# joesound212985/Deepfake-Detection-using-CLIP-Based-SigLIP-2-Vision-Transformers

Hardware: AMD Instinct MI355X
Metric: images/sec (train fwd+bwd) SigLIP-2-so400m@384 bf16 (higher is better)
Workload: dtype bf16; 1 GPU; so400m-patch14-384 encoder+pool-head train fwd+bwd, 384x384, per-GPU batch 128, seeded random weights; global_batch=128, parallelism=dp1

## Files before the change

### deepfake-detection-using-clip-based-siglip-2-vision-transformers_amd/csrc/attention.hip

```cpp
#include <stdlib.h>

#include "common.hip.h"
#include "kernels.h"

namespace sgl {

hipError_t attn_f32_fwd(const float*, const float*, const float*, float*, float*, int, int, int, int, int, int, hipStream_t);
hipError_t attn_f32_bwd(const float*, const float*, const float*, const float*, const float*, const float*, float*,
                        float*, int, int, int, int, int, int, hipStream_t);
hipError_t attn_ref_fwd(const float*, const float*, const float*, float*, float*, int, int, int, int, int, int, hipStream_t);
hipError_t attn_ref_bwd(const float*, const float*, const float*, const float*, const float*, const float*, float*,
                        float*, int, int, int, int, int, int, hipStream_t);

template <int DP>
struct AttnCfg {
  static constexpr int KS = DP / 16;
  static constexpr int DT = (DP + 31) / 32;
  static constexpr int CPR = DP / 8;
  static constexpr int RSTR = DP * 2 + 16;
  static constexpr int TSTR = 192;
  static constexpr int DSTR = 208;
};

__device__ __forceinline__ u32x4 a_ldg(__amdgpu_buffer_rsrc_t r, uint32_t off) {
  return __builtin_amdgcn_raw_buffer_load_b128(r, off, 0, 0);
}
template <typename T>
__device__ __forceinline__ lo_x8<T> as_x8(u32x4 v) { return __builtin_bit_cast(lo_x8<T>, v); }
template <typename T>
__device__ __forceinline__ lo_x8<T> lds_row8(const char* p) { return *reinterpret_cast<const lo_x8<T>*>(p); }
template <typename T>
__device__ __forceinline__ lo_x4<T> lds_tr4(const char* p) { return lds_read_tr16<T>(p); }
template <typename T>
__device__ __forceinline__ lo_x8<T> lds_trfrag(const char* img, int stride, int kk, int dcol0, int lane) {
  const int g = lane >> 4, q = (lane >> 2) & 3, p = lane & 3;
  const char* a = img + (16 * kk + 4 * (g >> 1) + q) * stride + (dcol0 + 16 * (g & 1) + 4 * p) * 2;
  const lo_x4<T> lo = lds_tr4<T>(a);
  const lo_x4<T> hi = lds_tr4<T>(a + 8 * stride);
  return __builtin_shufflevector(lo, hi, 0, 1, 2, 3, 4, 5, 6, 7);
}
template <typename T>
__device__ __forceinline__ lo_x8<T> pack8(const f32x16& s, int base) {
  lo_x8<T> r;
#pragma unroll
  for (int j = 0; j < 8; ++j) r[j] = (T)s[base + j];
  return r;
}
__device__ __forceinline__ float fast_exp2(float x) { return __builtin_amdgcn_exp2f(x); }

__device__ __forceinline__ bool head_block(int nb, int BH, int& bh, int& xb) {
  const int pid = blockIdx.x, xcd = pid & 7, slot = pid >> 3;
  const int hq = slot / nb;
  bh = hq * 8 + xcd;
  xb = slot - hq * nb;
  return bh < BH;
}
static inline dim3 head_grid(int nb, int BH) { return dim3((unsigned)(8 * ((BH + 7) / 8) * nb)); }

struct HeadSrc {
  uint32_t rowbytes, nc, bytes;
  size_t base;
};
__device__ __forceinline__ HeadSrc head_src(int ld, int b, int hd, int H, int N, int dh, int DP) {
  HeadSrc r;
  if (ld > 0) {
    r.rowbytes = (uint32_t)ld * 2u;
    r.nc = (uint32_t)dh / 8u;
    r.bytes = (uint32_t)(((size_t)(N - 1) * ld + dh) * 2);
    r.base = (size_t)b * N * ld + (size_t)hd * dh;
  } else {
    r.rowbytes = (uint32_t)DP * 2u;
    r.nc = (uint32_t)DP / 8u;
    r.bytes = (uint32_t)((size_t)N * DP * 2);
    r.base = ((size_t)b * H + hd) * (size_t)N * DP;
  }
  return r;
}

#define MFMA32(a, b, c) mfma_32x32x16((a), (b), (c))

__device__ __forceinline__ void att_dma16(u32x4 desc, uint32_t lds_addr, uint32_t voff) {
  asm volatile("s_mov_b32 m0, %0\n\ts_nop 0\n\tbuffer_load_dwordx4 %1, %2, 0 offen lds" ::"s"(lds_addr), "v"(voff), "s"(desc)
               : "memory");
}
__device__ __forceinline__ void att_dma4(u32x4 desc, uint32_t lds_addr, uint32_t voff) {
  asm volatile("s_mov_b32 m0, %0\n\ts_nop 0\n\tbuffer_load_dword %1, %2, 0 offen lds" ::"s"(lds_addr), "v"(voff), "s"(desc)
               : "memory");
}
__device__ __forceinline__ u32x4 att_desc(const void* base, uint32_t bytes) {
  const uint64_t q = (uint64_t)base;
  return u32x4{(uint32_t)q, (uint32_t)(q >> 32) & 0xffffu, bytes, 0x00020000u};
}
__device__ __forceinline__ uint32_t att_chunk_off(int cidx, int rows, int SC, int NC, uint32_t rowbytes) {
  const int row = cidx / SC, col = cidx - row * SC;
  return (row < rows && col < NC) ? (uint32_t)row * rowbytes + (uint32_t)col * 16u : SGL_OOB;
}
#define SGL_ATT_WAIT_BARRIER(n)                                   \
  do {                                                            \
    asm volatile("s_waitcnt vmcnt(" #n ") lgkmcnt(0)" ::: "memory"); \
    __builtin_amdgcn_sched_barrier(0);                            \
    __builtin_amdgcn_s_barrier();                                 \
    __builtin_amdgcn_sched_barrier(0);                            \
    asm volatile("" ::: "memory");                                \
  } while (0)

template <typename T, int DP, bool TOK>
__global__ __launch_bounds__(256) __attribute__((amdgpu_waves_per_eu(3, 3))) void attn_fwd_kernel(const T* __restrict__ Q, const T* __restrict__ K,
                                                          const T* __restrict__ V, T* __restrict__ out,
                                                          float* __restrict__ lse, int B, int H, int N, int dh, int ld,
                                                          float c, float scale) {
  using C = AttnCfg<DP>;
  constexpr int KT = 64;
  constexpr int KBYTES = KT * C::RSTR, VBYTES = KT * C::TSTR, STAGE = KBYTES + VBYTES;
  constexpr int SCK = C::RSTR / 16, SCV = C::TSTR / 16;
  constexpr int NIK = KT * SCK / 64, NIV = KT * SCV / 64, NSLOT = NIK + NIV;
  constexpr int NPW = (NSLOT + 3) / 4;
  static_assert(KT * SCK % 64 == 0 && KT * SCV % 64 == 0, "whole DMA instructions per image");
  extern __shared__ __attribute__((aligned(16))) char smem[];
  const int t = threadIdx.x, lane = t & 63;
  const int w = __builtin_amdgcn_readfirstlane(t >> 6);
  int bh, xb;
  if (!head_block((N + 127) / 128, B * H, bh, xb)) return;
  const int b = bh / H, hd = bh - b * H;
  const int q0 = xb * 128 + w * 32;
  HeadSrc src = head_src(TOK ? ld : 0, b, hd, H, N, dh, DP);
  if constexpr (!TOK) {
    src.rowbytes = (uint32_t)DP * 2u;
    src.nc = (uint32_t)DP / 8u;
  }
  const __amdgpu_buffer_rsrc_t rq = make_rsrc(Q + src.base, src.bytes);
  const u32x4 dk_ = att_desc(K + src.base, src.bytes);
  const u32x4 dv_ = att_desc(V + src.base, src.bytes);
  const uint32_t lds0 = (uint32_t)(size_t)((SGL_LDS char*)smem);

  const int qi = lane & 31, hh = lane >> 5;
  lo_x8<T> qf[C::KS];
#pragma unroll
  for (int ks = 0; ks < C::KS; ++ks) {
    const uint32_t ch = (uint32_t)(2 * ks + hh);
    qf[ks] = as_x8<T>(a_ldg(rq, (q0 + qi < N && ch < src.nc) ? (uint32_t)(q0 + qi) * src.rowbytes + ch * 16u : SGL_OOB));
  }

  uint32_t voff[NPW];
#pragma unroll
  for (int j = 0; j < NPW; ++j) {
    const int sl = w + 4 * j;
    voff[j] = (sl < NIK) ? att_chunk_off(sl * 64 + lane, KT, SCK, (int)src.nc, src.rowbytes)
                         : att_chunk_off((sl - NIK) * 64 + lane, KT, SCV, (int)src.nc, src.rowbytes);
  }
  const uint32_t tile_adv = (uint32_t)KT * src.rowbytes;
  auto issue = [&](int stage) {
    const uint32_t sb = lds0 + (uint32_t)(stage * STAGE);
#pragma unroll
    for (int j = 0; j < NPW; ++j) {
      const int sl = w + 4 * j;
      if (sl < NSLOT) att_dma16(sl < NIK ? dk_ : dv_, sb + (uint32_t)sl * 1024u, voff[j]);
      voff[j] += tile_adv;
    }
  };

  float m_run = -INFINITY, l_run = 0.f;
  f32x16 o[C::DT];
#pragma unroll
  for (int dt = 0; dt < C::DT; ++dt)
#pragma unroll
    for (int r = 0; r < 16; ++r) o[dt][r] = 0.f;

  const int ntiles = (N + KT - 1) / KT;
#pragma unroll
  for (int ks = 0; ks < C::KS; ++ks) asm volatile("" ::"v"(qf[ks]));
  asm volatile("s_waitcnt vmcnt(0)" ::: "memory");
  issue(0);
  for (int tile = 0; tile < ntiles; ++tile) {
    const int cur = tile & 1;
    SGL_ATT_WAIT_BARRIER(0);
    if (tile + 1 < ntiles) issue(cur ^ 1);
    const char* kb = smem + cur * STAGE;
    const char* vb = kb + KBYTES;
    f32x16 s0, s1;
#pragma unroll
    for (int r = 0; r < 16; ++r) { s0[r] = 0.f; s1[r] = 0.f; }
#pragma unroll
    for (int ks = 0; ks < C::KS; ++ks) {
      const lo_x8<T> k0 = lds_row8<T>(kb + qi * C::RSTR + (16 * ks + 8 * hh) * 2);
      const lo_x8<T> k1 = lds_row8<T>(kb + (qi + 32) * C::RSTR + (16 * ks + 8 * hh) * 2);
      s0 = MFMA32(k0, qf[ks], s0);
      s1 = MFMA32(k1, qf[ks], s1);
    }
    if (tile == ntiles - 1) {
#pragma unroll
      for (int r = 0; r < 16; ++r) {
        const int key = tile * KT + (r & 3) + 8 * (r >> 2) + 4 * hh;
        if (key >= N) s0[r] = -INFINITY;
        if (key + 32 >= N) s1[r] = -INFINITY;
      }
    }
    float mx = s0[0];
#pragma unroll
    for (int r = 1; r < 16; ++r) mx = fmaxf(mx, s0[r]);
#pragma unroll
    for (int r = 0; r < 16; ++r) mx = fmaxf(mx, s1[r]);
    mx = fmaxf(mx, __shfl_xor(mx, 32, 64));
    const float m_new = fmaxf(m_run, mx);
    const bool grew = __any(m_new > m_run);
    const float alpha = grew ? fast_exp2(c * (m_run - m_new)) : 1.0f;
    const float mc = m_new * c;
    float rs = 0.f;
#pragma unroll
    for (int r = 0; r < 16; ++r) {
      s0[r] = fast_exp2(fmaf(s0[r], c, -mc));
      s1[r] = fast_exp2(fmaf(s1[r], c, -mc));
      rs += s0[r] + s1[r];
    }
    l_run = l_run * alpha + rs;
    m_run = m_new;
    if (grew) {
#pragma unroll
      for (int dt = 0; dt < C::DT; ++dt)
#pragma unroll
        for (int r = 0; r < 16; ++r) o[dt][r] *= alpha;
    }
    lo_x8<T> pb[4];
    pb[0] = pack8<T>(s0, 0);
    pb[1] = pack8<T>(s0, 8);
    pb[2] = pack8<T>(s1, 0);
    pb[3] = pack8<T>(s1, 8);
#pragma unroll
    for (int dt = 0; dt < C::DT; ++dt)
#pragma unroll
      for (int kk = 0; kk < 4; ++kk) o[dt] = MFMA32(lds_trfrag<T>(vb, C::TSTR, kk, dt * 32, lane), pb[kk], o[dt]);
  }
  const float l = l_run + __shfl_xor(l_run, 32, 64);
  const float inv = 1.0f / l;
  const int q = q0 + qi;
  if (q < N) {
    T* orow = out + ((size_t)b * N + q) * ((size_t)H * dh) + hd * dh;
#pragma unroll
    for (int dt = 0; dt < C::DT; ++dt)
#pragma unroll
      for (int g4 = 0; g4 < 4; ++g4) {
        const int d = dt * 32 + 8 * g4 + 4 * hh;
        if (d < dh) {
          lo_x4<T> v4;
#pragma unroll
          for (int r = 0; r < 4; ++r) v4[r] = (T)(o[dt][4 * g4 + r] * inv);
          *reinterpret_cast<lo_x4<T>*>(orow + d) = v4;
        }
      }
    if (hh == 0) lse[(size_t)bh * N + q] = m_run * scale + __logf(l);
  }
}

template <typename T, int DP, bool TOK>
__global__ __launch_bounds__(256, 2) void attn_bwd_kv_kernel(const T* __restrict__ Q, const T* __restrict__ K,
                                                             const T* __restrict__ V, const T* __restrict__ dO,
                                                             const float* __restrict__ aux, T* __restrict__ dqkv,
                                                             int B, int H, int N, int dh, int ld, float c, float scale) {
  using C = AttnCfg<DP>;
  constexpr int QT = 32;
  constexpr int SC = C::DSTR / 16;
  constexpr int NIS = (QT * SC + 63) / 64;
  constexpr int IMG = NIS * 1024;
  constexpr int STAGE = 2 * IMG + QT * 8;
  constexpr int NSLOT = 2 * NIS + 1;
  static_assert(NSLOT <= 16 && NSLOT > 12, "four DMA slots per wave (three for the last wave)");
  extern __shared__ __attribute__((aligned(16))) char smem[];
  const int t = threadIdx.x, lane = t & 63;
  const int w = __builtin_amdgcn_readfirstlane(t >> 6);
  int bh, xb;
  if (!head_block((N + 127) / 128, B * H, bh, xb)) return;
  const int b = bh / H, hd = bh - b * H;
  const int D = H * dh;
  const int key0 = xb * 128 + w * 32;
  HeadSrc src = head_src(TOK ? ld : 0, b, hd, H, N, dh, DP);
  if constexpr (!TOK) {
    src.rowbytes = (uint32_t)DP * 2u;
    src.nc = (uint32_t)DP / 8u;
  }
  const __amdgpu_buffer_rsrc_t rk = make_rsrc(K + src.base, src.bytes);
  const __amdgpu_buffer_rsrc_t rv = make_rsrc(V + src.base, src.bytes);
  const T* dOb = dO + (size_t)b * N * D + hd * dh;
  const u32x4 dq_ = att_desc(Q + src.base, src.bytes);
  const u32x4 ddo = att_desc(dOb, (uint32_t)(((size_t)(N - 1) * D + dh) * 2));
  const u32x4 dax = att_desc(aux + (size_t)bh * N * 2, (uint32_t)((size_t)N * 8));
  const uint32_t lds0 = (uint32_t)(size_t)((SGL_LDS char*)smem);

  const int li = lane & 31, hh = lane >> 5;
  lo_x8<T> kfr[C::KS], vfr[C::KS];
#pragma unroll
  for (int ks = 0; ks < C::KS; ++ks) {
    const uint32_t ch = (uint32_t)(2 * ks + hh);
    const uint32_t off = (key0 + li < N && ch < src.nc) ? (uint32_t)(key0 + li) * src.rowbytes + ch * 16u : SGL_OOB;
    kfr[ks] = as_x8<T>(a_ldg(rk, off));
    vfr[ks] = as_x8<T>(a_ldg(rv, off));
  }

  uint32_t voff[4], vadv[4];
  u32x4 dsc[3];
#pragma unroll
  for (int j = 0; j < 4; ++j) {
    const int sl = w + 4 * j;
    if (sl < NIS) {
      voff[j] = att_chunk_off(sl * 64 + lane, QT, SC, (int)src.nc, src.rowbytes);
      vadv[j] = (uint32_t)QT * src.rowbytes;
    } else if (sl < 2 * NIS) {
      voff[j] = att_chunk_off((sl - NIS) * 64 + lane, QT, SC, dh / 8, (uint32_t)D * 2u);
      vadv[j] = (uint32_t)(QT * D * 2);
    } else {
      voff[j] = (uint32_t)lane * 4u;
      vadv[j] = (uint32_t)(QT * 8);
    }
    if (j < 3) dsc[j] = (sl < NIS) ? dq_ : ddo;
  }
  auto issue1 = [&](int j, int stage) {
    const uint32_t sb = lds0 + (uint32_t)(stage * STAGE) + (uint32_t)w * 1024u;
    if (j < 3) {
      att_dma16(dsc[j], sb + (uint32_t)j * 4096u, voff[j]);
    } else {
      if (w < 2) att_dma16(ddo, sb + 3u * 4096u, voff[3]);
      else if (w == 2) att_dma4(dax, lds0 + (uint32_t)(stage * STAGE + 2 * IMG), voff[3]);
    }
    voff[j] += vadv[j];
  };
  auto issue = [&](int stage) {
#pragma unroll
    for (int j = 0; j < 4; ++j) issue1(j, stage);
  };

  f32x16 dk[C::DT], dv[C::DT];
#pragma unroll
  for (int dt = 0; dt < C::DT; ++dt)
#pragma unroll
    for (int r = 0; r < 16; ++r) { dk[dt][r] = 0.f; dv[dt][r] = 0.f; }

  const int ntiles = (N + QT - 1) / QT;
#pragma unroll
  for (int ks = 0; ks < C::KS; ++ks) asm volatile("" ::"v"(kfr[ks]), "v"(vfr[ks]));
  asm volatile("s_waitcnt vmcnt(0)" ::: "memory");
  issue(0);
  issue(1);
  int st = 0;
  for (int qt = 0; qt < ntiles; ++qt) {
    if (w == 3) SGL_ATT_WAIT_BARRIER(3); else SGL_ATT_WAIT_BARRIER(4);
    const int st_next = (st == 0) ? 2 : st - 1;
    const char* qimg = smem + st * STAGE;
    const char* dimg = qimg + IMG;
    const float* ld = reinterpret_cast<const float*>(qimg + 2 * IMG);
    st = (st == 2) ? 0 : st + 1;
    f32x16 S, dP;
#pragma unroll
    for (int r = 0; r < 16; ++r) { S[r] = 0.f; dP[r] = 0.f; }
    lo_x8<T> qa[C::KS], da[C::KS];
#pragma unroll
    for (int ks = 0; ks < C::KS; ++ks) {
      qa[ks] = lds_row8<T>(qimg + li * C::DSTR + (16 * ks + 8 * hh) * 2);
      da[ks] = lds_row8<T>(dimg + li * C::DSTR + (16 * ks + 8 * hh) * 2);
    }
#pragma unroll
    for (int ks = 0; ks < C::KS; ++ks) {
      S = MFMA32(qa[ks], kfr[ks], S);
      dP = MFMA32(da[ks], vfr[ks], dP);
    }
    if constexpr (C::KS == 5) {
      __builtin_amdgcn_sched_group_barrier(0x100, 4, 0);
#pragma unroll
      for (int i = 0; i < 6; ++i) {
        __builtin_amdgcn_sched_group_barrier(0x008, 1, 0);
        __builtin_amdgcn_sched_group_barrier(0x100, 1, 0);
      }
      __builtin_amdgcn_sched_group_barrier(0x008, 4, 0);
    }
    __builtin_amdgcn_sched_barrier(0);
    constexpr int NF = 2 * 2 * C::DT;
    lo_x8<T> fr[NF];
    auto frag = [&](int i) {
      const int which = i & 1, kk = (i >> 1) & 1, dt = i >> 2;
      return lds_trfrag<T>(which ? qimg : dimg, C::DSTR, kk, dt * 32, lane);
    };
    constexpr int PRE = NF < 2 ? NF : 2;
#pragma unroll
    for (int i = 0; i < PRE; ++i) fr[i] = frag(i);
    __builtin_amdgcn_sched_barrier(0);
#pragma unroll
    for (int g4 = 0; g4 < 4; ++g4) {
      const f32x4 A0 = *reinterpret_cast<const f32x4*>(ld + 2 * (8 * g4 + 4 * hh));
      const f32x4 A1 = *reinterpret_cast<const f32x4*>(ld + 2 * (8 * g4 + 4 * hh) + 4);
      const float L4[4] = {A0[0], A0[2], A1[0], A1[2]};
      const float D4[4] = {A0[1], A0[3], A1[1], A1[3]};
#pragma unroll
      for (int r3 = 0; r3 < 4; ++r3) {
        const int r = 4 * g4 + r3;
        const float p = fast_exp2(fmaf(S[r], c, L4[r3]));
        S[r] = p;
        dP[r] = p * fmaf(dP[r], scale, D4[r3]);
      }
    }
    lo_x8<T> pb[2], dsb[2];
    pb[0] = pack8<T>(S, 0);
    pb[1] = pack8<T>(S, 8);
    dsb[0] = pack8<T>(dP, 0);
    dsb[1] = pack8<T>(dP, 8);
    __builtin_amdgcn_sched_barrier(0);
#pragma unroll
    for (int i = 0; i < NF; ++i) {
      if (i + PRE < NF) fr[i + PRE] = frag(i + PRE);
      const int which = i & 1, kk = (i >> 1) & 1, dt = i >> 2;
      if (which) dk[dt] = MFMA32(fr[i], dsb[kk], dk[dt]);
      else dv[dt] = MFMA32(fr[i], pb[kk], dv[dt]);
      if (i % 3 == 1) issue1(i / 3, st_next);
      __builtin_amdgcn_sched_barrier(0);
    }
#pragma unroll
    for (int j = (NF + 1) / 3; j < 4; ++j) issue1(j, st_next);
  }
  asm volatile("s_waitcnt vmcnt(0)" ::: "memory");
  const int key = key0 + li;
  if (key < N) {
    T* krow = dqkv + ((size_t)b * N + key) * (3 * (size_t)D) + D + hd * dh;
    T* vrow = krow + D;
#pragma unroll
    for (int dt = 0; dt < C::DT; ++dt)
#pragma unroll
      for (int g4 = 0; g4 < 4; ++g4) {
        const int d = dt * 32 + 8 * g4 + 4 * hh;
        if (d < dh) {
          lo_x4<T> a, g;
#pragma unroll
          for (int r = 0; r < 4; ++r) {
            a[r] = (T)dk[dt][4 * g4 + r];
            g[r] = (T)dv[dt][4 * g4 + r];
          }
          *reinterpret_cast<lo_x4<T>*>(krow + d) = a;
          *reinterpret_cast<lo_x4<T>*>(vrow + d) = g;
        }
      }
  }
}

template <typename T, int DP, bool TOK>
__global__ __launch_bounds__(256, 2) void attn_bwd_q_kernel(const T* __restrict__ Q, const T* __restrict__ K,
                                                            const T* __restrict__ V, const T* __restrict__ O,
                                                            const T* __restrict__ dO, const float* __restrict__ lse,
                                                            float* __restrict__ aux, T* __restrict__ dqkv,
                                                            int B, int H, int N, int dh, int ld, float c, float scale) {
  using C = AttnCfg<DP>;
  constexpr int KT = 32;
  constexpr int SCK = C::DSTR / 16, SCV = C::RSTR / 16;
  constexpr int NIK = (KT * SCK + 63) / 64, NIV = (KT * SCV + 63) / 64;
  constexpr int KIMG = NIK * 1024, VIMG = NIV * 1024, STAGE = KIMG + VIMG;
  constexpr int NSLOT = NIK + NIV;
  static_assert(NSLOT <= 16, "at most four DMA slots per wave");
  constexpr float LOG2E = 1.4426950408889634f;
  extern __shared__ __attribute__((aligned(16))) char smem[];
  const int t = threadIdx.x, lane = t & 63;
  const int w = __builtin_amdgcn_readfirstlane(t >> 6);
  int bh, xb;
  if (!head_block((N + 127) / 128, B * H, bh, xb)) return;
  const int b = bh / H, hd = bh - b * H;
  const int D = H * dh;
  const int q0 = xb * 128 + w * 32;
  HeadSrc src = head_src(TOK ? ld : 0, b, hd, H, N, dh, DP);
  if constexpr (!TOK) {
    src.rowbytes = (uint32_t)DP * 2u;
    src.nc = (uint32_t)DP / 8u;
  }
  const __amdgpu_buffer_rsrc_t rq = make_rsrc(Q + src.base, src.bytes);
  const T* dOb = dO + (size_t)b * N * D + hd * dh;
  const __amdgpu_buffer_rsrc_t rdo = make_rsrc(dOb, (uint32_t)(((size_t)(N - 1) * D + dh) * 2));
  const u32x4 dk_ = att_desc(K + src.base, src.bytes);
  const u32x4 dv_ = att_desc(V + src.base, src.bytes);
  const uint32_t lds0 = (uint32_t)(size_t)((SGL_LDS char*)smem);

  const int li = lane & 31, hh = lane >> 5;
  const int q = q0 + li;
  lo_x8<T> qf[C::KS], dof[C::KS];
#pragma unroll
  for (int ks = 0; ks < C::KS; ++ks) {
    const int col = 16 * ks + 8 * hh;
    qf[ks] = as_x8<T>(a_ldg(rq, (q < N && (uint32_t)(col >> 3) < src.nc) ? (uint32_t)q * src.rowbytes + (uint32_t)col * 2u
                                                                           : SGL_OOB));
    dof[ks] = as_x8<T>(a_ldg(rdo, (q < N && col < dh) ? (uint32_t)(((size_t)q * D + col) * 2) : SGL_OOB));
  }
  float dl = 0.f;
  {
    const __amdgpu_buffer_rsrc_t ro = make_rsrc(O + (size_t)b * N * D + hd * dh, (uint32_t)(((size_t)(N - 1) * D + dh) * 2));
#pragma unroll
    for (int ks = 0; ks < C::KS; ++ks) {
      const int col = 16 * ks + 8 * hh;
      const lo_x8<T> of = as_x8<T>(a_ldg(ro, (q < N && col < dh) ? (uint32_t)(((size_t)q * D + col) * 2) : SGL_OOB));
#pragma unroll
      for (int j = 0; j < 8; ++j) dl = fmaf((float)of[j], (float)dof[ks][j], dl);
    }
    dl += __shfl_xor(dl, 32, 64);
  }
  const float Lq = (q < N) ? -lse[(size_t)bh * N + q] * LOG2E : -INFINITY;
  const float Dq = (q < N) ? -dl * scale : 0.f;
  if (q < N && hh == 0) *reinterpret_cast<float2*>(aux + 2 * ((size_t)bh * N + q)) = make_float2(Lq, Dq);

  uint32_t voff[4];
  u32x4 dsc[4];
  uint32_t ldst[4];
#pragma unroll
  for (int j = 0; j < 4; ++j) {
    const int sl = w + 4 * j;
    if (sl < NIK) {
      voff[j] = att_chunk_off(sl * 64 + lane, KT, SCK, (int)src.nc, src.rowbytes);
      dsc[j] = dk_;
      ldst[j] = (uint32_t)sl * 1024u;
    } else {
      voff[j] = att_chunk_off((sl - NIK) * 64 + lane, KT, SCV, (int)src.nc, src.rowbytes);
      dsc[j] = dv_;
      ldst[j] = (uint32_t)(KIMG + (sl - NIK) * 1024);
    }
  }
  auto issue1 = [&](int j, int stage) {
    if (w + 4 * j < NSLOT) att_dma16(dsc[j], lds0 + (uint32_t)(stage * STAGE) + ldst[j], voff[j]);
    voff[j] += (uint32_t)KT * src.rowbytes;
  };

  f32x16 dq[C::DT];
#pragma unroll
  for (int dt = 0; dt < C::DT; ++dt)
#pragma unroll
    for (int r = 0; r < 16; ++r) dq[dt][r] = 0.f;

  const int ntiles = (N + KT - 1) / KT;
#pragma unroll
  for (int ks = 0; ks < C::KS; ++ks) asm volatile("" ::"v"(qf[ks]), "v"(dof[ks]));
  asm volatile("" ::"v"(Lq), "v"(Dq));
  asm volatile("s_waitcnt vmcnt(0)" ::: "memory");
#pragma unroll
  for (int j = 0; j < 4; ++j) issue1(j, 0);
#pragma unroll
  for (int j = 0; j < 4; ++j) issue1(j, 1);
  int st = 0;
  for (int kt = 0; kt < ntiles; ++kt) {
    const int nw = (NSLOT - w + 3) / 4;
    if (nw >= 4) SGL_ATT_WAIT_BARRIER(4);
    else if (nw == 3) SGL_ATT_WAIT_BARRIER(3);
    else if (nw == 2) SGL_ATT_WAIT_BARRIER(2);
    else SGL_ATT_WAIT_BARRIER(1);
    const int st_next = (st == 0) ? 2 : st - 1;
    const char* kimg = smem + st * STAGE;
    const char* vimg = kimg + KIMG;
    st = (st == 2) ? 0 : st + 1;
    f32x16 S, dP;
#pragma unroll
    for (int r = 0; r < 16; ++r) { S[r] = 0.f; dP[r] = 0.f; }
    lo_x8<T> ka[C::KS], va[C::KS];
#pragma unroll
    for (int ks = 0; ks < C::KS; ++ks) {
      ka[ks] = lds_row8<T>(kimg + li * C::DSTR + (16 * ks + 8 * hh) * 2);
      va[ks] = lds_row8<T>(vimg + li * C::RSTR + (16 * ks + 8 * hh) * 2);
    }
#pragma unroll
    for (int ks = 0; ks < C::KS; ++ks) {
      S = MFMA32(ka[ks], qf[ks], S);
      dP = MFMA32(va[ks], dof[ks], dP);
    }
    if constexpr (C::KS == 5) {
      __builtin_amdgcn_sched_group_barrier(0x100, 6, 0);
#pragma unroll
      for (int i = 0; i < 4; ++i) {
        __builtin_amdgcn_sched_group_barrier(0x008, 1, 0);
        __builtin_amdgcn_sched_group_barrier(0x100, 1, 0);
      }
      __builtin_amdgcn_sched_group_barrier(0x008, 6, 0);
    }
    __builtin_amdgcn_sched_barrier(0);
    lo_x8<T> kt_frag[C::DT][2];
#pragma unroll
    for (int dt = 0; dt < C::DT; ++dt)
#pragma unroll
      for (int kk = 0; kk < 2; ++kk) kt_frag[dt][kk] = lds_trfrag<T>(kimg, C::DSTR, kk, dt * 32, lane);
    __builtin_amdgcn_sched_barrier(0);
#pragma unroll
    for (int r = 0; r < 16; ++r) {
      const float p = fast_exp2(fmaf(S[r], c, Lq));
      dP[r] = p * fmaf(dP[r], scale, Dq);
    }
    if (kt == ntiles - 1) {
#pragma unroll
      for (int r = 0; r < 16; ++r) {
        const int key = kt * KT + (r & 3) + 8 * (r >> 2) + 4 * hh;
        if (key >= N) dP[r] = 0.f;
      }
    }
    lo_x8<T> dsb[2];
    dsb[0] = pack8<T>(dP, 0);
    dsb[1] = pack8<T>(dP, 8);
#pragma unroll
    for (int i = 0; i < 2 * C::DT; ++i) {
      dq[i >> 1] = MFMA32(kt_frag[i >> 1][i & 1], dsb[i & 1], dq[i >> 1]);
      if (i < 4) issue1(i, st_next);
      __builtin_amdgcn_sched_barrier(0);
    }
#pragma unroll
    for (int j = 2 * C::DT; j < 4; ++j) issue1(j, st_next);
  }
  asm volatile("s_waitcnt vmcnt(0)" ::: "memory");
  if (q < N) {
    T* qrow = dqkv + ((size_t)b * N + q) * (3 * (size_t)D) + hd * dh;
#pragma unroll
    for (int dt = 0; dt < C::DT; ++dt)
#pragma unroll
      for (int g4 = 0; g4 < 4; ++g4) {
        const int d = dt * 32 + 8 * g4 + 4 * hh;
        if (d < dh) {
          lo_x4<T> a;
#pragma unroll
          for (int r = 0; r < 4; ++r) a[r] = (T)dq[dt][4 * g4 + r];
          *reinterpret_cast<lo_x4<T>*>(qrow + d) = a;
        }
      }
  }
}

template <typename T, int DP>
static hipError_t fwd_launch(const T* q, const T* k, const T* v, T* out, float* lse, int B, int H, int N,
                             int dh, int ld, hipStream_t s) {
  using C = AttnCfg<DP>;
  constexpr int smem = 2 * (64 * C::RSTR + 64 * C::TSTR);
  const float scale = 1.0f / sqrtf((float)dh);
  if (ld > 0)
    hipLaunchKernelGGL((attn_fwd_kernel<T, DP, true>), head_grid((N + 127) / 128, B * H), dim3(256), smem, s, q, k, v, out, lse,
                       B, H, N, dh, ld, scale * 1.4426950408889634f, scale);
  else
    hipLaunchKernelGGL((attn_fwd_kernel<T, DP, false>), head_grid((N + 127) / 128, B * H), dim3(256), smem, s, q, k, v, out,
                       lse, B, H, N, dh, 0, scale * 1.4426950408889634f, scale);
  return hipGetLastError();
}

template <typename T, int DP>
static hipError_t bwd_launch(const T* q, const T* k, const T* v, const T* out, const T* dout,
                             const float* lse, T* dqkv, float* delta, int B, int H, int N, int dh, int ld,
                             hipStream_t s) {
  using C = AttnCfg<DP>;
  const float scale = 1.0f / sqrtf((float)dh);
  const float c = scale * 1.4426950408889634f;
  constexpr int smem_kv = 3 * (2 * ((32 * (C::DSTR / 16) + 63) / 64) * 1024 + 32 * 8);
  constexpr int smem_q = 3 * (((32 * (C::DSTR / 16) + 63) / 64) + ((32 * (C::RSTR / 16) + 63) / 64)) * 1024;
  const dim3 grid = head_grid((N + 127) / 128, B * H), block(256);
  if (ld > 0)
    hipLaunchKernelGGL((attn_bwd_q_kernel<T, DP, true>), grid, block, smem_q, s, q, k, v, out, dout, lse, delta, dqkv, B, H, N,
                       dh, ld, c, scale);
  else
    hipLaunchKernelGGL((attn_bwd_q_kernel<T, DP, false>), grid, block, smem_q, s, q, k, v, out, dout, lse, delta, dqkv, B, H, N,
                       dh, 0, c, scale);
  hipError_t e = hipGetLastError();
  if (e != hipSuccess) return e;
  if (ld > 0)
    hipLaunchKernelGGL((attn_bwd_kv_kernel<T, DP, true>), grid, block, smem_kv, s, q, k, v, dout, delta, dqkv, B, H, N, dh, ld, c,
                       scale);
  else
    hipLaunchKernelGGL((attn_bwd_kv_kernel<T, DP, false>), grid, block, smem_kv, s, q, k, v, dout, delta, dqkv, B, H, N, dh, 0,
                       c, scale);
  return hipGetLastError();
}

static bool attn_shape_ok(int N, int dh, int DP, int H, int ld) {
  if (dh % 8 || DP != ((dh + 15) / 16) * 16) return false;
  if (DP != 16 && DP != 32 && DP != 48 && DP != 64 && DP != 80 && DP != 96) return false;
  if (ld < 0 || (ld > 0 && (ld % 8 || ld < H * dh))) return false;
  if ((size_t)N * (ld > 0 ? ld : DP) * 2 >= (1ull << 31)) return false;
  if ((size_t)N * H * dh * 2 >= (1ull << 31)) return false;
  return true;
}

hipError_t attn_fwd(const void* q, const void* k, const void* v, int dtype, void* out, float* lse, int B, int H, int N,
                    int dh, int DP, int ld, hipStream_t s) {
  if (B * H == 0 || N == 0) return hipSuccess;
  if (dtype == DT_F32)
    return attn_ref_fwd((const float*)q, (const float*)k, (const float*)v, (float*)out, lse, B, H, N, dh, DP, ld, s);
  if (dtype == DT_F32_MFMA)
    return attn_f32_fwd((const float*)q, (const float*)k, (const float*)v, (float*)out, lse, B, H, N, dh, DP, ld, s);
  if (!attn_shape_ok(N, dh, DP, H, ld)) return hipErrorInvalidValue;
  if ((((uintptr_t)q) | ((uintptr_t)k) | ((uintptr_t)v)) & 15) return hipErrorInvalidValue;
#define SGL_F(T, DPV) \
  case DPV: return fwd_launch<T, DPV>((const T*)q, (const T*)k, (const T*)v, (T*)out, lse, B, H, N, dh, ld, s);
  if (dtype == DT_F16) {
    switch (DP) {
      SGL_F(f16, 16) SGL_F(f16, 32) SGL_F(f16, 48) SGL_F(f16, 64) SGL_F(f16, 80) SGL_F(f16, 96)
    }
    return hipErrorInvalidValue;
  }
  switch (DP) {
    SGL_F(bf16, 16) SGL_F(bf16, 32) SGL_F(bf16, 48) SGL_F(bf16, 64) SGL_F(bf16, 80) SGL_F(bf16, 96)
  }
#undef SGL_F
  return hipErrorInvalidValue;
}

hipError_t attn_bwd(const void* q, const void* k, const void* v, const void* out, const void* dout, const float* lse,
                    int dtype, void* dqkv, float* delta, float* , int B, int H, int N, int dh, int DP,
                    int ld, hipStream_t s) {
  if (B * H == 0 || N == 0) return hipSuccess;
  if (dtype == DT_F32)
    return attn_ref_bwd((const float*)q, (const float*)k, (const float*)v, (const float*)out, (const float*)dout, lse,
                        (float*)dqkv, delta, B, H, N, dh, DP, ld, s);
  if (dtype == DT_F32_MFMA)
    return attn_f32_bwd((const float*)q, (const float*)k, (const float*)v, (const float*)out, (const float*)dout, lse,
                        (float*)dqkv, delta, B, H, N, dh, DP, ld, s);
  if (!attn_shape_ok(N, dh, DP, H, ld)) return hipErrorInvalidValue;
  if ((((uintptr_t)q) | ((uintptr_t)k) | ((uintptr_t)v)) & 15) return hipErrorInvalidValue;
#define SGL_B(T, DPV)                                                                                  \
  case DPV:                                                                                            \
    return bwd_launch<T, DPV>((const T*)q, (const T*)k, (const T*)v, (const T*)out, (const T*)dout, lse, \
                              (T*)dqkv, delta, B, H, N, dh, ld, s);
  if (dtype == DT_F16) {
    switch (DP) {
      SGL_B(f16, 16) SGL_B(f16, 32) SGL_B(f16, 48) SGL_B(f16, 64) SGL_B(f16, 80) SGL_B(f16, 96)
    }
    return hipErrorInvalidValue;
  }
  switch (DP) {
    SGL_B(bf16, 16) SGL_B(bf16, 32) SGL_B(bf16, 48) SGL_B(bf16, 64) SGL_B(bf16, 80) SGL_B(bf16, 96)
  }
#undef SGL_B
  return hipErrorInvalidValue;
}

}
```

Baseline: 429.8 images/sec.

## Swizzle dual-use LDS images in attention backward and regroup DMA slot issue

Replaces the padded 208-byte-stride LDS image used for Q/dO and K tiles in the backward kernels with a 192-byte-stride image whose 16-byte chunks are XOR-swizzled by row. Both row reads and transposed reads go through precomputed per-lane offsets. This shrinks LDS per stage and is meant to avoid bank conflicts without padding. The forward kernel's DMA issue is regrouped so each wave issues K then V slots with compile-time predicates. The backward waits are rewritten around fixed slot counts, and the tail masking now uses a scalar remaining-key count. It risks incorrect swizzle indexing and wait-count mismatches.

```diff
diff --git a/deepfake-detection-using-clip-based-siglip-2-vision-transformers_amd/csrc/attention.hip b/deepfake-detection-using-clip-based-siglip-2-vision-transformers_amd/csrc/attention.hip
--- a/deepfake-detection-using-clip-based-siglip-2-vision-transformers_amd/csrc/attention.hip
+++ b/deepfake-detection-using-clip-based-siglip-2-vision-transformers_amd/csrc/attention.hip
@@ -1,5 +1,6 @@
 #include <stdlib.h>
 
+#include "attn_lds_layout.h"
 #include "common.hip.h"
 #include "kernels.h"
 
@@ -19,7 +20,6 @@
   static constexpr int CPR = DP / 8;
   static constexpr int RSTR = DP * 2 + 16;
   static constexpr int TSTR = 192;
-  static constexpr int DSTR = 208;
 };
 
 __device__ __forceinline__ u32x4 a_ldg(__amdgpu_buffer_rsrc_t r, uint32_t off) {
@@ -37,6 +37,16 @@
   const char* a = img + (16 * kk + 4 * (g >> 1) + q) * stride + (dcol0 + 16 * (g & 1) + 4 * p) * 2;
   const lo_x4<T> lo = lds_tr4<T>(a);
   const lo_x4<T> hi = lds_tr4<T>(a + 8 * stride);
+  return __builtin_shufflevector(lo, hi, 0, 1, 2, 3, 4, 5, 6, 7);
+}
+template <typename T>
+__device__ __forceinline__ lo_x8<T> dual_row8(const char* img, AttDualRow ro, int ks) {
+  return lds_row8<T>(img + att_dual_row_byte(ro, ks));
+}
+template <typename T>
+__device__ __forceinline__ lo_x8<T> dual_trfrag(const char* img, AttDualTr tr, int kk, int dt) {
+  const lo_x4<T> lo = lds_tr4<T>(img + att_dual_tr_byte(tr.lo, kk, dt));
+  const lo_x4<T> hi = lds_tr4<T>(img + att_dual_tr_byte(tr.hi, kk, dt));
   return __builtin_shufflevector(lo, hi, 0, 1, 2, 3, 4, 5, 6, 7);
 }
 template <typename T>
@@ -91,9 +101,18 @@
   const uint64_t q = (uint64_t)base;
   return u32x4{(uint32_t)q, (uint32_t)(q >> 32) & 0xffffu, bytes, 0x00020000u};
 }
+static_assert(ATT_OOB == SGL_OOB, "one out-of-range offset");
 __device__ __forceinline__ uint32_t att_chunk_off(int cidx, int rows, int SC, int NC, uint32_t rowbytes) {
   const int row = cidx / SC, col = cidx - row * SC;
   return (row < rows && col < NC) ? (uint32_t)row * rowbytes + (uint32_t)col * 16u : SGL_OOB;
+}
+template <int N>
+__device__ __forceinline__ void att_wait_barrier() {
+  asm volatile("s_waitcnt vmcnt(%0) lgkmcnt(0)" ::"n"(N) : "memory");
+  __builtin_amdgcn_sched_barrier(0);
+  __builtin_amdgcn_s_barrier();
+  __builtin_amdgcn_sched_barrier(0);
+  asm volatile("" ::: "memory");
 }
 #define SGL_ATT_WAIT_BARRIER(n)                                   \
   do {                                                            \
@@ -114,8 +133,9 @@
   constexpr int KBYTES = KT * C::RSTR, VBYTES = KT * C::TSTR, STAGE = KBYTES + VBYTES;
   constexpr int SCK = C::RSTR / 16, SCV = C::TSTR / 16;
   constexpr int NIK = KT * SCK / 64, NIV = KT * SCV / 64, NSLOT = NIK + NIV;
-  constexpr int NPW = (NSLOT + 3) / 4;
+  constexpr int NPK = (NIK + 3) / 4, NPV = (NIV + 3) / 4, NPW = NPK + NPV;
   static_assert(KT * SCK % 64 == 0 && KT * SCV % 64 == 0, "whole DMA instructions per image");
+  static_assert(KBYTES == NIK * 1024 && VBYTES == NIV * 1024, "the images are their DMA instructions, back to back");
   extern __shared__ __attribute__((aligned(16))) char smem[];
   const int t = threadIdx.x, lane = t & 63;
   const int w = __builtin_amdgcn_readfirstlane(t >> 6);
@@ -143,18 +163,20 @@
 
   uint32_t voff[NPW];
 #pragma unroll
-  for (int j = 0; j < NPW; ++j) {
-    const int sl = w + 4 * j;
-    voff[j] = (sl < NIK) ? att_chunk_off(sl * 64 + lane, KT, SCK, (int)src.nc, src.rowbytes)
-                         : att_chunk_off((sl - NIK) * 64 + lane, KT, SCV, (int)src.nc, src.rowbytes);
-  }
+  for (int j = 0; j < NPW; ++j)
+    voff[j] = (j < NPK) ? att_chunk_off((w + 4 * j) * 64 + lane, KT, SCK, (int)src.nc, src.rowbytes)
+                        : att_chunk_off((w + 4 * (j - NPK)) * 64 + lane, KT, SCV, (int)src.nc, src.rowbytes);
   const uint32_t tile_adv = (uint32_t)KT * src.rowbytes;
   auto issue = [&](int stage) {
-    const uint32_t sb = lds0 + (uint32_t)(stage * STAGE);
+    const uint32_t sb = lds0 + (uint32_t)(stage * STAGE) + (uint32_t)w * 1024u;
 #pragma unroll
     for (int j = 0; j < NPW; ++j) {
-      const int sl = w + 4 * j;
-      if (sl < NSLOT) att_dma16(sl < NIK ? dk_ : dv_, sb + (uint32_t)sl * 1024u, voff[j]);
+      if (j < NPK) {
+        if (4 * j + 3 < NIK || w + 4 * j < NIK) att_dma16(dk_, sb + (uint32_t)(4 * j) * 1024u, voff[j]);
+      } else {
+        const int jv = j - NPK;
+        if (4 * jv + 3 < NIV || w + 4 * jv < NIV) att_dma16(dv_, sb + (uint32_t)(KBYTES + 4 * jv * 1024), voff[j]);
+      }
       voff[j] += tile_adv;
     }
   };
@@ -188,11 +210,13 @@
       s1 = MFMA32(k1, qf[ks], s1);
     }
     if (tile == ntiles - 1) {
+      int nrem = N - tile * KT;
+      asm volatile("" : "+s"(nrem));
 #pragma unroll
       for (int r = 0; r < 16; ++r) {
-        const int key = tile * KT + (r & 3) + 8 * (r >> 2) + 4 * hh;
-        if (key >= N) s0[r] = -INFINITY;
-        if (key + 32 >= N) s1[r] = -INFINITY;
+        const int kr = (r & 3) + 8 * (r >> 2) + 4 * hh;
+        if (kr >= nrem) s0[r] = -INFINITY;
+        if (kr + 32 >= nrem) s1[r] = -INFINITY;
       }
     }
     float mx = s0[0];
@@ -258,12 +282,13 @@
                                                              int B, int H, int N, int dh, int ld, float c, float scale) {
   using C = AttnCfg<DP>;
   constexpr int QT = 32;
-  constexpr int SC = C::DSTR / 16;
-  constexpr int NIS = (QT * SC + 63) / 64;
-  constexpr int IMG = NIS * 1024;
+  static_assert(QT == ATT_DUAL_ROWS && C::DT * 4 <= ATT_DUAL_SLOTS, "the dual-use image holds one tile");
+  constexpr int NIS = ATT_DUAL_NDMA;
+  constexpr int IMG = ATT_DUAL_BYTES;
   constexpr int STAGE = 2 * IMG + QT * 8;
   constexpr int NSLOT = 2 * NIS + 1;
-  static_assert(NSLOT <= 16 && NSLOT > 12, "four DMA slots per wave (three for the last wave)");
+  static_assert(NSLOT <= 16 && NSLOT > 12, "four DMA slots per wave");
+  static_assert(NSLOT == 13, "slot 12, the pair slot, is wave 0's fourth: the waits below count on it");
   extern __shared__ __attribute__((aligned(16))) char smem[];
   const int t = threadIdx.x, lane = t & 63;
   const int w = __builtin_amdgcn_readfirstlane(t >> 6);
@@ -286,6 +311,8 @@
   const uint32_t lds0 = (uint32_t)(size_t)((SGL_LDS char*)smem);
 
   const int li = lane & 31, hh = lane >> 5;
+  const AttDualRow rof = att_dual_row_lane(lane);
+  const AttDualTr tr = att_dual_tr_lane(lane);
   lo_x8<T> kfr[C::KS], vfr[C::KS];
 #pragma unroll
   for (int ks = 0; ks < C::KS; ++ks) {
@@ -301,10 +328,10 @@
   for (int j = 0; j < 4; ++j) {
     const int sl = w + 4 * j;
     if (sl < NIS) {
-      voff[j] = att_chunk_off(sl * 64 + lane, QT, SC, (int)src.nc, src.rowbytes);
+      voff[j] = att_dual_dma_src(sl, lane, QT, (int)src.nc, src.rowbytes);
       vadv[j] = (uint32_t)QT * src.rowbytes;
     } else if (sl < 2 * NIS) {
-      voff[j] = att_chunk_off((sl - NIS) * 64 + lane, QT, SC, dh / 8, (uint32_t)D * 2u);
+      voff[j] = att_dual_dma_src(sl - NIS, lane, QT, dh / 8, (uint32_t)D * 2u);
       vadv[j] = (uint32_t)(QT * D * 2);
     } else {
       voff[j] = (uint32_t)lane * 4u;
@@ -317,8 +344,7 @@
     if (j < 3) {
       att_dma16(dsc[j], sb + (uint32_t)j * 4096u, voff[j]);
     } else {
-      if (w < 2) att_dma16(ddo, sb + 3u * 4096u, voff[3]);
-      else if (w == 2) att_dma4(dax, lds0 + (uint32_t)(stage * STAGE + 2 * IMG), voff[3]);
+      if (w == 0) att_dma4(dax, lds0 + (uint32_t)(stage * STAGE + 2 * IMG), voff[3]);
     }
     voff[j] += vadv[j];
   };
@@ -341,7 +367,7 @@
   issue(1);
   int st = 0;
   for (int qt = 0; qt < ntiles; ++qt) {
-    if (w == 3) SGL_ATT_WAIT_BARRIER(3); else SGL_ATT_WAIT_BARRIER(4);
+    if (w == 0) SGL_ATT_WAIT_BARRIER(4); else SGL_ATT_WAIT_BARRIER(3);
     const int st_next = (st == 0) ? 2 : st - 1;
     const char* qimg = smem + st * STAGE;
     const char* dimg = qimg + IMG;
@@ -353,8 +379,8 @@
     lo_x8<T> qa[C::KS], da[C::KS];
 #pragma unroll
     for (int ks = 0; ks < C::KS; ++ks) {
-      qa[ks] = lds_row8<T>(qimg + li * C::DSTR + (16 * ks + 8 * hh) * 2);
-      da[ks] = lds_row8<T>(dimg + li * C::DSTR + (16 * ks + 8 * hh) * 2);
+      qa[ks] = dual_row8<T>(qimg, rof, ks);
+      da[ks] = dual_row8<T>(dimg, rof, ks);
     }
 #pragma unroll
     for (int ks = 0; ks < C::KS; ++ks) {
@@ -375,7 +401,7 @@
     lo_x8<T> fr[NF];
     auto frag = [&](int i) {
       const int which = i & 1, kk = (i >> 1) & 1, dt = i >> 2;
-      return lds_trfrag<T>(which ? qimg : dimg, C::DSTR, kk, dt * 32, lane);
+      return dual_trfrag<T>(which ? qimg : dimg, tr, kk, dt);
     };
     constexpr int PRE = NF < 2 ? NF : 2;
 #pragma unroll
@@ -445,11 +471,13 @@
                                                             int B, int H, int N, int dh, int ld, float c, float scale) {
   using C = AttnCfg<DP>;
   constexpr int KT = 32;
-  constexpr int SCK = C::DSTR / 16, SCV = C::RSTR / 16;
-  constexpr int NIK = (KT * SCK + 63) / 64, NIV = (KT * SCV + 63) / 64;
+  static_assert(KT == ATT_DUAL_ROWS && C::DT * 4 <= ATT_DUAL_SLOTS, "the dual-use image holds one tile");
+  constexpr int SCV = C::RSTR / 16;
+  constexpr int NIK = ATT_DUAL_NDMA, NIV = (KT * SCV + 63) / 64;
   constexpr int KIMG = NIK * 1024, VIMG = NIV * 1024, STAGE = KIMG + VIMG;
   constexpr int NSLOT = NIK + NIV;
   static_assert(NSLOT <= 16, "at most four DMA slots per wave");
+  constexpr int JF = NSLOT / 4, REM = NSLOT % 4;
   constexpr float LOG2E = 1.4426950408889634f;
   extern __shared__ __attribute__((aligned(16))) char smem[];
   const int t = threadIdx.x, lane = t & 63;
@@ -472,6 +500,8 @@
   const uint32_t lds0 = (uint32_t)(size_t)((SGL_LDS char*)smem);
 
   const int li = lane & 31, hh = lane >> 5;
+  const AttDualRow rof = att_dual_row_lane(lane);
+  const AttDualTr tr = att_dual_tr_lane(lane);
   const int q = q0 + li;
   lo_x8<T> qf[C::KS], dof[C::KS];
 #pragma unroll
@@ -504,7 +534,7 @@
   for (int j = 0; j < 4; ++j) {
     const int sl = w + 4 * j;
     if (sl < NIK) {
-      voff[j] = att_chunk_off(sl * 64 + lane, KT, SCK, (int)src.nc, src.rowbytes);
+      voff[j] = att_dual_dma_src(sl, lane, KT, (int)src.nc, src.rowbytes);
       dsc[j] = dk_;
       ldst[j] = (uint32_t)sl * 1024u;
     } else {
@@ -514,7 +544,7 @@
     }
   }
   auto issue1 = [&](int j, int stage) {
-    if (w + 4 * j < NSLOT) att_dma16(dsc[j], lds0 + (uint32_t)(stage * STAGE) + ldst[j], voff[j]);
+    if (j < JF || (j == JF && w < REM)) att_dma16(dsc[j], lds0 + (uint32_t)(stage * STAGE) + ldst[j], voff[j]);
     voff[j] += (uint32_t)KT * src.rowbytes;
   };
 
@@ -535,11 +565,8 @@
   for (int j = 0; j < 4; ++j) issue1(j, 1);
   int st = 0;
   for (int kt = 0; kt < ntiles; ++kt) {
-    const int nw = (NSLOT - w + 3) / 4;
-    if (nw >= 4) SGL_ATT_WAIT_BARRIER(4);
-    else if (nw == 3) SGL_ATT_WAIT_BARRIER(3);
-    else if (nw == 2) SGL_ATT_WAIT_BARRIER(2);
-    else SGL_ATT_WAIT_BARRIER(1);
+    if (REM != 0 && w < REM) att_wait_barrier<JF + 1>();
+    else att_wait_barrier<JF>();
     const int st_next = (st == 0) ? 2 : st - 1;
     const char* kimg = smem + st * STAGE;
     const char* vimg = kimg + KIMG;
@@ -550,7 +577,7 @@
     lo_x8<T> ka[C::KS], va[C::KS];
 #pragma unroll
     for (int ks = 0; ks < C::KS; ++ks) {
-      ka[ks] = lds_row8<T>(kimg + li * C::DSTR + (16 * ks + 8 * hh) * 2);
+      ka[ks] = dual_row8<T>(kimg, rof, ks);
       va[ks] = lds_row8<T>(vimg + li * C::RSTR + (16 * ks + 8 * hh) * 2);
     }
 #pragma unroll
@@ -572,7 +599,7 @@
 #pragma unroll
     for (int dt = 0; dt < C::DT; ++dt)
 #pragma unroll
-      for (int kk = 0; kk < 2; ++kk) kt_frag[dt][kk] = lds_trfrag<T>(kimg, C::DSTR, kk, dt * 32, lane);
+      for (int kk = 0; kk < 2; ++kk) kt_frag[dt][kk] = dual_trfrag<T>(kimg, tr, kk, dt);
     __builtin_amdgcn_sched_barrier(0);
 #pragma unroll
     for (int r = 0; r < 16; ++r) {
@@ -638,8 +665,8 @@
   using C = AttnCfg<DP>;
   const float scale = 1.0f / sqrtf((float)dh);
   const float c = scale * 1.4426950408889634f;
-  constexpr int smem_kv = 3 * (2 * ((32 * (C::DSTR / 16) + 63) / 64) * 1024 + 32 * 8);
-  constexpr int smem_q = 3 * (((32 * (C::DSTR / 16) + 63) / 64) + ((32 * (C::RSTR / 16) + 63) / 64)) * 1024;
+  constexpr int smem_kv = 3 * (2 * ATT_DUAL_BYTES + 32 * 8);
+  constexpr int smem_q = 3 * (ATT_DUAL_BYTES + ((32 * (C::RSTR / 16) + 63) / 64) * 1024);
   const dim3 grid = head_grid((N + 127) / 128, B * H), block(256);
   if (ld > 0)
     hipLaunchKernelGGL((attn_bwd_q_kernel<T, DP, true>), grid, block, smem_q, s, q, k, v, out, dout, lse, delta, dqkv, B, H, N,
diff --git a/deepfake-detection-using-clip-based-siglip-2-vision-transformers_amd/csrc/attn_lds_layout.h b/deepfake-detection-using-clip-based-siglip-2-vision-transformers_amd/csrc/attn_lds_layout.h
--- /dev/null
+++ b/deepfake-detection-using-clip-based-siglip-2-vision-transformers_amd/csrc/attn_lds_layout.h
@@ -0,0 +1,45 @@
+#pragma once
+#include <stdint.h>
+
+#if defined(__HIPCC__)
+#define SGL_HD __host__ __device__ inline
+#else
+#define SGL_HD inline
+#endif
+
+namespace sgl {
+
+constexpr int ATT_DUAL_ROWS = 32;
+constexpr int ATT_DUAL_SLOTS = 12;
+constexpr int ATT_DUAL_STRIDE = ATT_DUAL_SLOTS * 16;
+constexpr int ATT_DUAL_BYTES = ATT_DUAL_ROWS * ATT_DUAL_STRIDE;
+constexpr int ATT_DUAL_NDMA = ATT_DUAL_BYTES / 1024;
+constexpr uint32_t ATT_OOB = 0x80000000u;
+
+SGL_HD int att_dual_swz(int row, int chunk) { return chunk ^ ((row >> 2) & 3); }
+
+SGL_HD uint32_t att_dual_dma_src(int inst, int lane, int rows, int nc, uint32_t rowbytes) {
+  const int cidx = inst * 64 + lane;
+  const int row = cidx / ATT_DUAL_SLOTS, slot = cidx - row * ATT_DUAL_SLOTS;
+  const int col = att_dual_swz(row, slot);
+  return (row < rows && col < nc) ? (uint32_t)row * rowbytes + (uint32_t)col * 16u : ATT_OOB;
+}
+
+SGL_HD int att_dual_chunk_byte(int row, int chunk) { return row * ATT_DUAL_STRIDE + att_dual_swz(row, chunk) * 16; }
+
+struct AttDualRow { int even, odd; };
+SGL_HD AttDualRow att_dual_row_lane(int lane) {
+  const int r = lane & 31, h = lane >> 5;
+  return AttDualRow{att_dual_chunk_byte(r, h), att_dual_chunk_byte(r, 2 + h) - 32};
+}
+SGL_HD int att_dual_row_byte(AttDualRow a, int ks) { return ((ks & 1) ? a.odd : a.even) + 32 * ks; }
+
+struct AttDualTr { int lo, hi; };
+SGL_HD AttDualTr att_dual_tr_lane(int lane) {
+  const int g = lane >> 4, q = (lane >> 2) & 3, p = lane & 3;
+  const int row = 4 * (g >> 1) + q, chunk = 2 * (g & 1) + (p >> 1), sub = 8 * (p & 1);
+  return AttDualTr{att_dual_chunk_byte(row, chunk) + sub, att_dual_chunk_byte(row + 8, chunk) + sub};
+}
+SGL_HD int att_dual_tr_byte(int lane_off, int kk, int dt) { return lane_off + kk * 16 * ATT_DUAL_STRIDE + dt * 64; }
+
+}
```

Result: no change. 431.6 images/sec (median of 4 runs) (+0.4%).
